# agordon/fastx_toolkit

Measured on AMD Instinct MI355X. Metric: Mreads/s (150 bp) quality-trim+filter, higher is better.
Workload: dtype u8

## Files before the change

fastx_toolkit_amd/csrc/fxg_device.h:

```cpp
#pragma once
#include <hip/hip_runtime.h>
#include <stdint.h>
#include <cstdio>
#include <cstring>

#include "../../include/fxg.h"

typedef unsigned int       u32;
typedef unsigned long long u64;
typedef unsigned int u32x4 __attribute__((ext_vector_type(4)));

#define FXG_HD __host__ __device__ __forceinline__
#define FXG_PLAN_FAIL(...) do { snprintf(err, cap, __VA_ARGS__); return FXG_E_INVALID; } while (0)
static inline int fxg_text_check_len(unsigned long long text_len, char *err, size_t cap) { if (text_len > 0xFFFFFFF0ull) FXG_PLAN_FAIL("text block too large (%llu bytes)", text_len); return FXG_OK; }
static inline bool fxg_text_lpr_ok(int lpr) { return lpr == 4 || lpr == 2; }

#if defined(FXG_ABLATION) || defined(FXG_DBG_BITS)
#define FXG_DBG(a, bit) ((a).debug & (bit))
#else
#define FXG_DBG(a, bit) 0u
#endif

#define FXG_BLOCK 256
#define FXG_WAVES (FXG_BLOCK / 64)
#ifndef FXG_TBLOCK
#define FXG_TBLOCK 256
#endif
#define FXG_TWAVES (FXG_TBLOCK / 64)
#ifndef FXG_CLIP_GATHER_K
#define FXG_CLIP_GATHER_K 4
#endif
#ifndef FXG_CLIP_DEPTH
#define FXG_CLIP_DEPTH 4u
#endif
#define FXG_CK_SLOTS 7u
#ifndef FXG_CLIP_TBLOCK
#define FXG_CLIP_TBLOCK 256
#endif
#define FXG_MAX_TILE FXG_TBLOCK
#define FXG_TICKET_GROUPS 8
#define FXG_TICKET_STRIDE 32
#define FXG_CTRL_WORDS 64

struct FxgKArgs {
    const uint8_t  *bases;
    const uint8_t  *qual;
    const uint16_t *len;
    u64  n;
// ... 37 lines not shown
    int  ft_first, ft_last;
    u32  ft_trim_end, ft_min_len;
    u32  mask_char;
    u32  nf_keep_n;
    u32  rev_dw;
    u64 *extra;
    const uint8_t  *clip_src;
    u64  clip_total;
    u32  clip_stride;
    const uint16_t *wlen;
    float *clip_ck;
    u32  clip_ck_rows;
    u32  clip_ptab_rows;
    u32  clip_ptab_stride;
    u32  clip_ptab_cols;
    u32  clip_ptab_dia1;
    char adapter[100];
    uint8_t clip_ptab_row[256];
};

__device__ __forceinline__ u32 fxg_lane() { return threadIdx.x & 63u; }

FXG_HD u32 fxg_ge_flags(u32 w, u32 K) { return (((w & 0x7f7f7f7fu) + K) | w) & 0x80808080u; }

FXG_HD u32 fxg_pack4(u32 f)
{
    u32 t = f >> 7;
    t |= t >> 7;
    t |= t >> 14;
    return t & 0xFu;
// ... 552 lines not shown
```

fastx_toolkit_amd/csrc/fxg_engine_clip.hip:

```cpp
#include "fxg_host.h"

#define FXG_CLIP_CASE_PACKED(N) case -N: return fxg_launch_tiles(c, (pl.ka.clip_global ? fxg_kernel_tiles<-N, 0, true> : fxg_kernel_tiles<-N, 0, false>), pl, ctr);
#define FXG_CLIP_CASE_GENERAL(N) case N: return fxg_launch_tiles(c, fxg_kernel_tiles<N, 0>, pl, ctr);
#define FXG_CLIP_DEFINE_UNIT(K) \
    int FXG_CLIP_UNIT_FN(K)(fxg_ctx *c, FxgPlan &pl, u64 *ctr) { switch (pl.amax) { FXG_CLIP_UNIT(K)(FXG_CLIP_CASE_PACKED, FXG_CLIP_CASE_GENERAL) default: return FXG_CLIP_NOT_MINE; } }

#ifdef FXG_CLIP_TU
FXG_CLIP_DEFINE_UNIT(FXG_CLIP_TU)
#else
FXG_CLIP_FOR_UNITS(FXG_CLIP_DEFINE_UNIT)
#endif
```

fastx_toolkit_amd/csrc/fxg_kernels.h:

```cpp
#pragma once
#include "fxg_device.h"
#include "fxg_clip_instances.h"

#define FXG_INVALID_TUPLE 0xFFFFFFFFu

#define FXG_NTALLY 16
struct FxgLds {
    u32 slot_bytes, so_ksrc, so_kidx, so_ktab;
    u32 off_scratch, off_tally, off_bm_g, off_bm_l, off_bases, off_ptab, total;
    u32 has_tab;
};
__host__ __device__ inline u32 fxg_r16(u32 x) { return (x + 15u) & ~15u; }
__host__ __device__ inline FxgLds fxg_lds_layout(u32 T, u32 stride, u32 bitmaps, u32 stage_stride, u32 nslots = 2, bool no_tab = false, u32 ptab_bytes = 0u)
{
    FxgLds l;
    l.so_ksrc = fxg_r16((T + 1) * 4);
    l.so_kidx = l.so_ksrc + fxg_r16(T * 4);
    l.so_ktab = l.so_kidx + fxg_r16(T * 2);
    l.has_tab = (stage_stride || no_tab) ? 0u : 1u;
    l.slot_bytes = l.so_ktab + (l.has_tab ? fxg_r16(((T * stride + 15) / 16 + 1) * 2) : 0u);
    u32 o = nslots * l.slot_bytes;
    l.off_scratch = o; o += fxg_r16(48 * 4);
    l.off_tally = o;   o += FXG_NTALLY * 8;
    const u32 words = (T * stride + 31) / 32 + 2;
    l.off_bm_g = o;    o += bitmaps ? fxg_r16(words * 4) * (bitmaps == 4u ? 4u : 1u) : 0;
    l.off_bm_l = bitmaps == 1u ? l.off_bm_g : o;    o += bitmaps == 2u ? fxg_r16(words * 4) : 0;
    l.off_bases = o;   o += stage_stride ? fxg_r16(T * stage_stride + 16) : 0;
    l.off_ptab = o;    o += fxg_r16(ptab_bytes);
    l.total = o;
    return l;
}

FXG_HD u32 fxg_bitmap_count(const FxgKArgs &a, bool use_q, bool clip) { return !use_q ? 0u : (clip && a.tq == a.fq) ? 1u : 2u; }

#ifdef FXG_HOST_EMULATION
FXG_HD int fxg_wave_max(int n) { return n; }
#else
__device__ __forceinline__ int fxg_wave_max(int n)
{
    int v = n;
#pragma unroll
    for (int d = 1; d < 64; d <<= 1) { const int o = __shfl_xor(v, d, 64); v = o > v ? o : v; }
// ... 111 lines not shown
#define FXG_PTAB_MAX_ROWS_K 8u

FXG_HD void fxg_ptab_row_map(const char *adapter, int alen, uint8_t (&row)[256])
{
    for (int b = 0; b < 256; ++b) row[b] = 0u;
    row[0] = 0x80u;
    u32 next = 2u;
    for (int t = 0; t < alen; ++t) {
        const u32 c = (u32)(uint8_t)adapter[t];
        if (c == (u32)'N' || row[c] != 0u) continue;
        row[c] = (uint8_t)(0x80u | next++);
    }
    row[(u32)'N'] = 0x80u | 1u;
}

FXG_HD void fxg_clip_ptab_build(const FxgKArgs &a, uint8_t *ptab, u32 tid, u32 nthreads)
{
    uint16_t *lut = reinterpret_cast<uint16_t *>(ptab);
    const int COLS = (int)a.clip_ptab_cols, A = a.alen < COLS ? a.alen : COLS;
    const u32 R = a.clip_ptab_rows, ST = a.clip_ptab_stride;
    for (u32 b = tid; b < 256u; b += nthreads) {
        const u32 e = a.clip_ptab_row[b], row = e & 0x7Fu;
        lut[b] = (uint16_t)(FXG_PTAB_LUT_BYTES + row * ST);
        if (e & 0x80u) {
            float *pv = reinterpret_cast<float *>(ptab + FXG_PTAB_LUT_BYTES + row * ST);
            u32 *sv = reinterpret_cast<u32 *>(ptab + FXG_PTAB_LUT_BYTES + (R + row) * ST);
            for (int t = 0; t < COLS; ++t) {
                const u32 tc = t < A ? (u32)(uint8_t)a.adapter[t] : 0u;
                const bool eq = tc == b, qn = b == (u32)'N', tn = tc == (u32)'N';
                pv[t] = tn ? (qn ? 0.0f : 0.1f) : (qn ? 0.1f : (eq ? 1.0f : -1.0f));
                sv[t] = (tn || qn) ? 0u : a.clip_ptab_dia1 + (eq ? 1u : 0u);
            }
        }
    }
}

#ifndef FXG_HOST_EMULATION
#define FXG_SCHED_FENCE() __builtin_amdgcn_sched_barrier(0)
// ... 119 lines not shown
#else
            const u32 w = reinterpret_cast<const u32 *>(rd)[k];
#endif
            const u32 v = w ^ 0x4E4E4E4Eu;
            const u32 z = (v - 0x01010101u) & ~v & 0x80808080u;
            const int pos = 4 * k + (int)((u32)__builtin_ctz(z | 0x80000000u) >> 3);
            first_n = (z != 0u && pos < len) ? pos : first_n;
        }
    } else {
#pragma unroll 1
        for (int k = len_u - 1; k >= 0; --k) first_n = (k < len && rd[k] == (uint8_t)'N') ? k : first_n;
    }
    return first_n;
}

template <int AMAX, bool GL = false>
FXG_HD int fxg_clip_two_pass(const FxgKArgs &a, const uint8_t *rd, int len, int rows, float &best, u32 &bw, u32 &bq, int &first_n, const bool UR = false, const uint8_t *ptab = nullptr)
{
    constexpr int C = FxgClip2<AMAX>::C;
    float S[AMAX], Sm[AMAX], P0[AMAX], P1[AMAX], P2[AMAX], CB[AMAX];
    const int A = a.alen;
#pragma unroll
    for (int t = 0; t < AMAX; ++t) { S[t] = (t <= 3) ? 0.0f : -5.0f * (float)(t - 3); Sm[t] = S[t] + -5.0f; P0[t] = P1[t] = P2[t] = CB[t] = S[t]; }
    const int early_rows = (A - 4 < rows) ? (A - 4 > 0 ? A - 4 : 0) : rows;
    const int rows_u = UR ? rows : fxg_wave_max(rows > 0 ? rows : 0);
    if (rows_u <= 0) return 0;
    float b1 = -1000000.0f;
    int q = 0, r0 = 0, bq1 = 0;
    u32 cn = 0u, gw0 = 0u, gw1 = 0u;
    int gmax = 0;
    u32 pr[16] = {}, st[16] = {}, on = 0u;
    const u32 step_off = a.clip_ptab_rows * a.clip_ptab_stride;
    const uint16_t *lut = reinterpret_cast<const uint16_t *>(ptab);
    if constexpr (GL) {
        gmax = fxg_gl_last_dword(a.clip_total, (u64)(rd - a.clip_src));
        gw0 = fxg_ld32(rd, 0, gmax); gw1 = fxg_ld32(rd, 1, gmax);
        on = lut[(gw0 >> 8) & 0xFFu];
        fxg_ptab_fetch<AMAX, false>(ptab, lut[gw0 & 0xFFu], step_off, pr, st);
    } else {
        const u32 o0 = lut[rd[0]];
        on = lut[rd[1]]; cn = rd[2];
        fxg_ptab_fetch<AMAX, false>(ptab, o0, step_off, pr, st);
    }
#define FXG_CLIP_CHUNK(EARLY, Psave, Pwin)                                                                                   \
    {                                                                                                                        \
        _Pragma("unroll") for (int t = 0; t < AMAX; ++t) Psave[t] = S[t];                                                    \
        const int q0 = q, qend = q + C < rows_u ? q + C : rows_u;                                                            \
        bool upd = false;                                                                                                    \
        _Pragma("unroll 1") for (; q < qend; ++q) {                                                                          \
            float rm;                                                                                                        \
            if constexpr (GL) {                   \
                const u32 ca = ((((q + 2) >> 2) == (q >> 2) ? gw0 : gw1) >> ((u32)((q + 2) & 3) << 3)) & 0xFFu;             \
                const u32 on2 = lut[ca];                                                                                     \
                if ((q & 3) == 3) { gw0 = gw1; gw1 = fxg_ld32(rd, (q >> 2) + 2, gmax); }                                     \
                if (!UR && q >= rows) continue;                                                                              \
                rm = fxg_clip_row_score_t<AMAX, EARLY>(A, q, S, Sm, pr, st, ptab, on, step_off);                             \
                on = on2;                                                                                                    \
            } else {                                                                                                         \
                if (!UR && q >= rows) continue;           \
                const u32 on2 = lut[cn];                                                                                     \
                cn = rd[q + 3];                                                                                              \
                rm = fxg_clip_row_score_t<AMAX, EARLY>(A, q, S, Sm, pr, st, ptab, on, step_off);                             \
                on = on2;                                                                                                    \
            }                                                                                                                \
            const bool g = rm > b1;                                                                                          \
            b1 = g ? rm : b1; bq1 = g ? q : bq1; upd = upd || g;                                                             \
        }                                                                                                                    \
        if (upd) {                                                                                                           \
            _Pragma("unroll") for (int t = 0; t < AMAX; ++t) CB[t] = Pwin[t];                                                \
            r0 = q0 - 2 * C > 0 ? q0 - 2 * C : 0;                                                                            \
        }                                                                                                                    \
    }
    static_assert(2 * C >= AMAX - 4, "early rows must end inside the first two chunks");
    FXG_CLIP_CHUNK(true, P0, P1)
    if (q < rows_u) FXG_CLIP_CHUNK(true, P1, P2)
    while (q < rows_u) {
// ... 1 lines not shown
        if (q >= rows_u) break;
        FXG_CLIP_CHUNK(false, P0, P1)
        if (q >= rows_u) break;
        FXG_CLIP_CHUNK(false, P1, P2)
    }
#undef FXG_CLIP_CHUNK
    if (rows <= 0) return 0;
    if (FXG_DBG(a, 32u)) { best = b1; bq = (u32)bq1; bw = 0u; return 0; }
    u32 W[AMAX];
#pragma unroll
    for (int t = 0; t < AMAX; ++t) { S[t] = CB[t]; Sm[t] = CB[t] + -5.0f; W[t] = ((u32)(t + 1) << 19) + FXG_PK_SZ1; }
    q = r0;
    constexpr int SPAN = FxgClip2<AMAX>::SPAN;
    const int rs = bq1 - SPAN + 1 > r0 ? bq1 - SPAN + 1 : r0;
    const int qlast = rows - 1;
#define FXG_RD_AHEAD(i) rd[GL && (i) > qlast ? qlast : (i)]
    {
        const u32 o0 = lut[rd[q]];
        on = lut[FXG_RD_AHEAD(q + 1)]; cn = FXG_RD_AHEAD(q + 2);
        fxg_ptab_fetch<AMAX, true>(ptab, o0, step_off, pr, st);
    }
    const int n0 = rs - r0, n0u = fxg_wave_max(n0);
#pragma unroll 1
    for (int i = 0; i < n0u; ++i) {
        if (i >= n0) continue;
        const u32 on2 = lut[cn];
        cn = FXG_RD_AHEAD(q + 3);
        (void)fxg_clip_row_score_t<AMAX, true, true>(A, q, S, Sm, pr, st, ptab, on, step_off);
        on = on2; ++q;
    }
    const int win = bq1 - rs, n1 = win < early_rows ? win : early_rows, n2 = win - n1;
    const int n1u = fxg_wave_max(n1), n2u = fxg_wave_max(n2);
#pragma unroll 1
    for (int i = 0; i < n1u; ++i) {
        if (i >= n1) continue;
        const u32 on2 = lut[cn];
        cn = FXG_RD_AHEAD(q + 3);
        fxg_clip_row_packed_t<AMAX, true, false>(A, q, (u32)(q - rs), S, Sm, W, best, bw, bq, pr, st, ptab, on, step_off);
        on = on2; ++q;
    }
#pragma unroll 1
    for (int i = 0; i < n2u; ++i) {
        if (i >= n2) continue;
        const u32 on2 = lut[cn];
        cn = FXG_RD_AHEAD(q + 3);
        fxg_clip_row_packed_t<AMAX, false, false>(A, q, (u32)(q - rs), S, Sm, W, best, bw, bq, pr, st, ptab, on, step_off);
        on = on2; ++q;
    }
    fxg_clip_row_packed_t<AMAX, true, true>(A, bq1, (u32)(bq1 - rs), S, Sm, W, best, bw, bq, pr, st, ptab, on, step_off);
#undef FXG_RD_AHEAD
    if (!(a.clip_flags & FXG_CLIP_KEEP_N)) first_n = fxg_clip_first_n(rd, len, UR ? len : fxg_wave_max(len), a.clip_stride, first_n);
    return rs;
}

#define FXG_K_MAT1 1u
#define FXG_K_DIA1 (1u << 7)
#define FXG_K_SZ1  (1u << 14)
#define FXG_K_START(v) ((u32)(v) << 23)
__host__ __device__ constexpr int fxg_clip_k_amin(int amax) { return amax <= 16 ? 1 : fxg_clip_bucket_below(amax) + 1; }
static_assert(fxg_clip_k_amin(16) == 1 && fxg_clip_k_amin(20) == 17 && fxg_clip_k_amin(24) == 21 && fxg_clip_k_amin(64) == 61 && fxg_clip_k_amin(72) == 65 &&
              fxg_clip_k_amin(88) == 81 && fxg_clip_k_amin(100) == 89, "a bucket's smallest adapter is the next smaller bucket + 1");
template <int AMAX> struct FxgClipK { static constexpr bool SM = AMAX <= 24; static constexpr int NSM = SM ? AMAX : 1; };

template <int AMAX, bool EARLY, bool TRACK>
FXG_HD void fxg_clip_row_kt(const FxgKArgs &a, int A, u32 c, int q, u32 vstart, float (&S)[AMAX], float (&Sm)[FxgClipK<AMAX>::NSM], u32 (&W)[AMAX],
                            float &best, u32 &bw, u32 &bq, const uint8_t *ptab)
// ... 213 lines not shown
        ++q;
    }
#pragma unroll 1
    for (int i = 0; i < n2u; ++i) {
        if (i >= n2) continue;
        fxg_clip_row_k<AMAX, false, false>(a, A, (u32)rd[q], q, (u32)(q - r0), S, Sk, W, best, bw, bq, ptab);
        ++q;
    }
    fxg_clip_row_k<AMAX, true, true>(a, A, (u32)rd[bq1], bq1, (u32)(bq1 - r0), S, Sk, W, best, bw, bq, ptab);
    if (!(a.clip_flags & FXG_CLIP_KEEP_N)) {
        first_n = fxg_clip_first_n(rd, len, UR ? len : fxg_wave_max(len), a.clip_stride, first_n);
    }
    return r0;
}

template <int AMAX, bool KFORM, bool GL = false>
FXG_HD void fxg_clip_read_packed(const FxgKArgs &a, const uint8_t *rd, int len, int rows,
                                 u32 *out_len, u32 *keep, u32 *reason, u32 *clipped, u32 *adapter_only, float *ck = nullptr, u32 cks = 0u, const bool UR = false,
                                 const uint8_t *ptab = nullptr)
{
    float best = -1000000.0f;
    u32 bw = FXG_INVALID_TUPLE, bq = 0u;
    int first_n = len, qbase = 0;
    if constexpr (!KFORM) qbase = fxg_clip_two_pass<AMAX, GL>(a, rd, len, rows, best, bw, bq, first_n, UR, ptab);
    if constexpr (KFORM) {
        int r0 = 0;
        if (ck) r0 = fxg_clip_two_pass_k<AMAX, GL>(a, rd, len, rows, ck, cks, best, bw, bq, first_n, UR, ptab);
        else fxg_clip_rows_k<AMAX>(a, rd, len, rows, best, bw, bq, first_n, UR, ptab);
        const int v = (int)(bw >> 23), matches = (int)(bw & 127u), diag = (int)((bw >> 7) & 127u);
        fxg_clip_finish(a, len, v < 256 ? r0 + v : 0, v < 256 ? 0 : v - 256, diag - matches, (int)((bw >> 14) & 511u), matches,
                        (int)bq, first_n, out_len, keep, reason, clipped, adapter_only);
        return;
    }
    const int matches = (int)(bw & 31u), diag = (int)((bw >> 14) & 31u);
    fxg_clip_finish(a, len, qbase + (int)(bw >> 24), (int)((bw >> 19) & 31u), diag - matches, (int)((bw >> 5) & 511u), matches,
                    (int)bq, first_n, out_len, keep, reason, clipped, adapter_only);
}

struct FxgCounts {
// ... 86 lines not shown
    for (u32 c = tid; c < nchunks; c += nthreads) {
        const u32 o = c << 4;
        const u64 at = tb + o;
        u32x4 v;
        if ((at & 15u) == 0u) v = fxg_window(src, (long long)at, total, 0, (int)(tbytes - o < 16u ? tbytes - o : 16u));
        else {
            u64 lo = 0, hi = 0;
            const int nb = (int)(tbytes - o < 16u ? tbytes - o : 16u);
            for (int i = 0; i < nb; ++i) { const u64 b = src[at + i]; if (i < 8) lo |= b << (8 * i); else hi |= b << (8 * (i - 8)); }
            v = (u32x4){(u32)lo, (u32)(lo >> 32), (u32)hi, (u32)(hi >> 32)};
        }
        *reinterpret_cast<u32x4 *>(sb + o) = v;
    }
}

__host__ __device__ constexpr int fxg_clip_cols(int amax) { return -amax; }
__host__ __device__ constexpr bool fxg_clip_kform(int amax) { return amax < -16; }
template <int AMAX, bool GL = false>
FXG_HD u32 fxg_decide_a(const FxgKArgs &a, const u32 *bm_g, const u32 *bm_l, const uint8_t *sb, u32 r0, u32 tid,
                        u32 *keep_out, u32 *len_out, float *ck = nullptr, u32 cks = 0u, const uint8_t *ptab = nullptr)
{
    const u32 stride = a.stride;
    const u32 rl = a.len ? (u32)a.len[r0 + tid] : a.fixed_len;
    u32 reason = FXG_R_KEPT, clipped = 0, keep = 1, curlen = rl, ao = 0;
    const int rows = a.wlen ? (int)a.wlen[r0 + tid] : (int)rl;
    if constexpr (AMAX > 0) fxg_clip_read<AMAX>(a, sb + tid * a.clip_stride, (int)rl, rows, &curlen, &keep, &reason, &clipped, &ao, !a.len && !a.wlen);
    if constexpr (AMAX < 0) {
        constexpr int COLS = fxg_clip_cols(AMAX);
        constexpr bool KF = fxg_clip_kform(AMAX);
        const uint8_t *rd = GL ? a.clip_src + (u64)(r0 + tid) * a.clip_stride : sb + tid * a.clip_stride;
        if (!a.len && !a.wlen) fxg_clip_read_packed<COLS, KF, GL>(a, rd, (int)a.fixed_len, (int)a.fixed_len, &curlen, &keep, &reason, &clipped, &ao, ck, cks, true, ptab);
        else fxg_clip_read_packed<COLS, KF, GL>(a, rd, (int)rl, rows, &curlen, &keep, &reason, &clipped, &ao, ck, cks, false, ptab);
    }
    if (keep && (a.stages & FXG_STAGE_QTRIM)) {
        const u32 k = fxg_bits_last(bm_g, tid * stride, curlen);
        curlen = k;
        if (!(k > 0 && (int)k >= a.qt_min_len)) { keep = 0; reason = FXG_R_QTRIM; }
    }
    if (keep && (a.stages & FXG_STAGE_QFILTER)) {
        const u32 low = bm_l == bm_g ? curlen - fxg_bits_count(bm_g, tid * stride, curlen) : fxg_bits_count(bm_l, tid * stride, curlen);
        int n0 = (int)curlen * a.qf_keep_pct / 100;
        if (n0 < 0) n0 = 0;
        if (a.qf_drop_all || (int)low > n0) { keep = 0; reason = FXG_R_QFILTER; }
    }
    const u32 w = (curlen & 0xFFFFu) | (keep << 16) | (reason << 17) | (clipped << 21) | (ao << FXG_RES_ADAPTER_ONLY_BIT);
    a.res[r0 + tid] = w;
    *keep_out = keep; *len_out = curlen;
// ... 150 lines not shown
#ifndef FXG_PRIO_WRITEOUT
#define FXG_PRIO_WRITEOUT 3
#endif
#ifndef FXG_PRIO_STAGING
#define FXG_PRIO_STAGING 2
#endif
#ifndef FXG_CLIP_WAVES_WIDE
#define FXG_CLIP_WAVES_WIDE 2
#endif
#ifdef FXG_CLIP_WAVES_ALL
__host__ __device__ constexpr int fxg_clip_waves(int amax) { return amax > 0 ? 1 : FXG_CLIP_WAVES_ALL; }
#else
__host__ __device__ constexpr int fxg_clip_waves(int amax) { return amax > 0 ? 1 : fxg_clip_cols(amax) <= 36 ? FXG_CLIP_WAVES : fxg_clip_cols(amax) <= 64 ? 3 : FXG_CLIP_WAVES_WIDE; }
#endif
template <int AMAX, int MODE> struct FxgTileBlock { static constexpr int threads = (MODE == 0 && AMAX < 0 && AMAX >= -16) ? FXG_CLIP_TBLOCK : FXG_TBLOCK; };
template <int AMAX, int MODE, bool GL = false>
__global__ __launch_bounds__((FxgTileBlock<AMAX, MODE>::threads), (AMAX == 0 ? FXG_MIN_WAVES : fxg_clip_waves(AMAX))) void fxg_kernel_tiles(const FxgKArgs a)
{
    extern __shared__ __attribute__((aligned(16))) unsigned char smem[];
    constexpr bool REV = (MODE == 2 || MODE == 5);
    constexpr u32 TB = (u32)FxgTileBlock<AMAX, MODE>::threads, TW = TB / 64u;
    const u32 T = a.tile_reads, stride = a.stride, tid = threadIdx.x;
    const bool use_q = (MODE == 0 && (a.stages & (FXG_STAGE_QTRIM | FXG_STAGE_QFILTER)) != 0) || MODE == 3;
    const u32 NSLOT = (MODE == 0 && AMAX != 0) ? a.depth : 2u;
    constexpr bool PTAB = MODE == 0 && fxg_clip_uses_ptab(AMAX);
    const FxgLds L = fxg_lds_layout(T, stride, MODE == 4 ? 4u : fxg_bitmap_count(a, use_q, MODE == 0 && AMAX != 0), (MODE == 0 && AMAX != 0) ? (GL ? 0u : a.clip_stride) : 0u, NSLOT, MODE == 0 && AMAX != 0, PTAB ? fxg_ptab_bytes(a.clip_ptab_rows, a.clip_ptab_stride) : 0u);
    u32 m_reads = 0, m_nt = 0, art_bad = 0;
    u32 *bm_g = reinterpret_cast<u32 *>(smem + L.off_bm_g);
    u32 *bm_l = reinterpret_cast<u32 *>(smem + L.off_bm_l);
    uint8_t *sb = smem + L.off_bases;
    u32 *scratch = reinterpret_cast<u32 *>(smem + L.off_scratch);
    u32 *s_tot = scratch + 2 * TW, *s_ticket = s_tot + 8;
    u64 *bc = reinterpret_cast<u64 *>(s_tot + 10);
    u64 *tally = reinterpret_cast<u64 *>(smem + L.off_tally);
    if (tid < FXG_NTALLY) tally[tid] = 0ull;
    if constexpr (PTAB) fxg_clip_ptab_build(a, smem + L.off_ptab, tid, TB);
#ifdef FXG_ABLATION
    u64 ph[8] = {0, 0, 0, 0, 0, 0, 0, 0}, pt = __builtin_amdgcn_s_memrealtime();
    const u64 clk_t0 = __builtin_amdgcn_s_memtime(), clk_r0 = __builtin_amdgcn_s_memrealtime();
#define FXG_TPHASE(i) do { const u64 now_ = __builtin_amdgcn_s_memrealtime(); ph[i] += now_ - pt; pt = now_; } while (0)
#else
#define FXG_TPHASE(i) do { } while (0)
#endif

    if (a.compact) {
        if (tid == 0) s_ticket[0] = atomicAdd(a.role, 1u);
        __syncthreads();
        const bool scanner = (s_ticket[0] == 0u);
        __syncthreads();
        if (scanner) { if (tid < 64) fxg_scanner(a); return; }
    }
// ... 7 lines not shown
    for (;;) {
        u64 peek = 0;
        if (tid < 64 && pend != FXG_NO_TILE && a.compact) peek = fxg_peek_prefix(a, pend);
        if (cur < a.ntiles) {
            constexpr bool TICKET_AFTER_DECISION = (MODE == 0 && AMAX != 0);
            if (!TICKET_AFTER_DECISION && tid == 0) s_ticket[tk ^ 1u] = atomicAdd(my_ticket, 1u);
            const u32 r0 = cur * T;
            const u64 left = a.n - (u64)r0;
            const u32 nreads = left < (u64)T ? (u32)left : T;
            const u64 tb = (u64)r0 * stride;
            const u32 tbytes = nreads * stride;
            unsigned char *sl = smem + slot * L.slot_bytes;
            if constexpr (MODE == 0 || MODE == 3 || MODE == 4) {
                if constexpr (MODE == 0 && AMAX != 0) __builtin_amdgcn_s_setprio(FXG_PRIO_STAGING);
                if (use_q && !FXG_DBG(a, 8u)) fxg_phase_bitmaps(a, tb, tbytes, bm_g, bm_l, tid, TB);
                if constexpr (MODE == 0 && AMAX != 0) { if (!GL && (!FXG_DBG(a, 16u) || pend == FXG_NO_TILE)) fxg_phase_stage_bases(a.clip_src, a.clip_total, (u64)r0 * a.clip_stride, nreads * a.clip_stride, sb, tid, TB); }
                if constexpr (MODE == 4) fxg_phase_census(a, tb, tbytes, fxg_census_bitmaps(bm_g, T, stride), tid, TB);
                __syncthreads();
                if constexpr (MODE == 0 && AMAX != 0) __builtin_amdgcn_s_setprio(0);
            }
            FXG_TPHASE(0);
            u32 keep = 0, olen = 0, anchor = tid * stride, word = 0;
            if (tid < nreads) {
                if constexpr (MODE == 0 && AMAX < -16) {
                    float *ck = a.clip_ck ? a.clip_ck + (size_t)blockIdx.x * ((size_t)FXG_CK_SLOTS * (u32)fxg_clip_cols(AMAX) * TB) + tid : nullptr;
                    word = fxg_decide_a<AMAX, GL>(a, bm_g, bm_l, sb, r0, tid, &keep, &olen, ck, TB, PTAB ? smem + L.off_ptab : nullptr);
                } else if constexpr (MODE == 0 && AMAX < 0) {
                    word = fxg_decide_a<AMAX, GL>(a, bm_g, bm_l, sb, r0, tid, &keep, &olen, nullptr, 0u, PTAB ? smem + L.off_ptab : nullptr);
                } else if constexpr (MODE == 0) word = fxg_decide_a<AMAX>(a, bm_g, bm_l, sb, r0, tid, &keep, &olen);
                else if constexpr (MODE == 3) { u32 nl; word = fxg_decide_mask(a, bm_l, r0, tid, &keep, &olen, &nl); m_nt += nl; m_reads += (nl != 0u); }
                else if constexpr (MODE == 4) word = fxg_decide_census(a, fxg_census_bitmaps(bm_g, T, stride), tid * stride, r0, tid, &keep, &olen, &art_bad);
                else word = fxg_decide_b<REV>(a, r0, tid, &keep, &olen, &anchor);
            }
#ifdef FXG_ABLATION
            {
                const u64 b0 = __builtin_amdgcn_s_memrealtime();
                __syncthreads();
                if ((tid & 63u) == 0u) atomicAdd(reinterpret_cast<u64 *>(a.errflag + 10) + 5, __builtin_amdgcn_s_memrealtime() - b0);
            }
#endif
            FXG_TPHASE(1);
            if (TICKET_AFTER_DECISION && tid == 0) s_ticket[tk ^ 1u] = atomicAdd(my_ticket, 1u);
            fxg_tile_tally<AMAX, MODE>(word, tid < nreads, tally);
// ... 151 lines not shown
```

fastx_toolkit_amd/csrc/fxg_plan.h:

```cpp
#pragma once
#include <cstdio>
#include <cstdlib>
#include <cstring>

#include "fxg_instances.h"
#include "fxg_knobs.h"

static_assert(fxg_clip_bucket(1) != 0 && fxg_clip_bucket(FXG_MAX_ADAPTER) != 0, "every adapter length the plan accepts needs a packed clip instance");

struct FxgPlan {
    FxgKArgs ka;
    bool group_a;
    bool clip, use_q, rev;
    bool mask, artifacts;
    int  inst;
    int  rows_nw;
    int  rows_h;
    int  amax;
    u32  lds;
    u32  block;
    u64  ck_per_wg;
};

static inline int fxg_clampi(long long v, int lo, int hi) { return v < lo ? lo : (v > hi ? hi : (int)v); }

static inline u32 fxg_pick_tile(u32 stride, bool clip, u32 block = FXG_TBLOCK, const FxgKnobs &kn = fxg_knobs_read(FXG_KNOBS_REQUEST))
{
    const u64 budget = clip ? 60ull * 1024 : 20ull * 1024;
    u32 T = block;
    if (kn.tile >= 1 && kn.tile <= (int)block && (kn.tile & (kn.tile - 1)) == 0) return (u32)kn.tile;
    while (T > 1 && (u64)T * stride > budget) T >>= 1;
    return T;
}

static inline FxgLds fxg_plan_layout(const FxgPlan *pl)
{
    const FxgKArgs &ka = pl->ka;
    return pl->group_a ? fxg_lds_layout(ka.tile_reads, ka.stride, fxg_bitmap_count(ka, pl->use_q, pl->clip), (pl->clip && !ka.clip_global) ? ka.clip_stride : 0u, pl->clip ? ka.depth : 2u, pl->clip,
                                        (pl->clip && fxg_clip_uses_ptab(pl->amax)) ? fxg_ptab_bytes(ka.clip_ptab_rows, ka.clip_ptab_stride) : 0u)
         : pl->mask ? fxg_lds_layout(ka.tile_reads, ka.stride, 2u, 0u)
         : pl->artifacts ? fxg_lds_layout(ka.tile_reads, ka.stride, 4u, 0u) : fxg_lds_layout(ka.tile_reads, ka.stride, 0u, 0u);
}
static inline u32 fxg_plan_lds(const FxgPlan *pl) { return fxg_plan_layout(pl).total; }

static inline int fxg_make_plan(const fxg_batch *in, const fxg_params *p, const fxg_out *out, FxgPlan *pl, char *err, size_t cap, u32 clip_stride = 0,
                                const FxgKnobs &kn = fxg_knobs_read(FXG_KNOBS_REQUEST))
{
    const u32 st = p->stages;
    const bool ga = (st & (FXG_STAGE_CLIP | FXG_STAGE_QTRIM | FXG_STAGE_QFILTER)) != 0;
    const bool gb = (st & (FXG_STAGE_REVCOMP | FXG_STAGE_FTRIM | FXG_STAGE_FTRIM_END)) != 0;
    const bool gm = (st & FXG_STAGE_MASK) != 0, gf = (st & (FXG_STAGE_ARTIFACTS | FXG_STAGE_NFILTER)) != 0;
    if ((int)ga + (int)gb + (int)gm + (int)gf != 1 || (st & (FXG_STAGE_ARTIFACTS | FXG_STAGE_NFILTER)) == (FXG_STAGE_ARTIFACTS | FXG_STAGE_NFILTER))
        FXG_PLAN_FAIL("unsupported stage chain 0x%x: use [CLIP][QTRIM][QFILTER], [REVCOMP][FTRIM|FTRIM_END], [MASK], [ARTIFACTS] or [NFILTER]", st);
    if (gm && !in->qual) FXG_PLAN_FAIL("fastq_masker needs qualities");
// ... 58 lines not shown
        ka.clip_ptab_dia1 = kform ? FXG_K_DIA1 : FXG_PK_DIA1;
        if (kform && ka.clip_ptab_rows > FXG_PTAB_MAX_ROWS_K) {
            pl->amax = ka.alen <= 32 ? 32 : ka.alen <= 64 ? 64 : 100;
            pl->ck_per_wg = 0;
        }
    }
    const u32 S = in->stride;
    const bool rows = ga && !pl->clip && ka.compact && kn.rows != 0 && S >= 28u && S <= (kn.rows >= 2 ? 304u : 208u);
    pl->inst = pl->clip ? FXG_INST_CLIP
             : rows ? (S <= 40u ? FXG_INST_MULTI4 : S <= 56u ? FXG_INST_MULTI3 : S < 80u ? FXG_INST_MULTI2
                       : S <= 104u ? FXG_INST_ROWS26 : S <= 152u ? FXG_INST_ROWS38 : S <= 208u ? FXG_INST_ROWS26X2 : FXG_INST_ROWS38X2)
             : ga ? FXG_INST_TILES00 : gm ? FXG_INST_TILES03 : gf ? FXG_INST_TILES04 : pl->rev ? FXG_INST_TILES02 : FXG_INST_TILES01;
    const FxgInstInfo ii = fxg_inst_info[pl->inst];
    pl->block = pl->clip ? fxg_tile_block(pl->amax, 0) : ii.block;
    pl->rows_nw = (int)ii.nw; pl->rows_h = (int)ii.h;
    ka.clip_global = 0u;
    u32 T = pl->rows_nw ? FXG_ROWS_T * ii.r / ii.h : fxg_pick_tile(pl->clip ? ka.clip_stride : in->stride, pl->clip, pl->block, kn);
    if (pl->clip && pl->amax < 0 && (pl->amax >= -16 || pl->ck_per_wg != 0) && clip_stride == 0u && (ka.clip_stride & 3u) == 0u && ((uintptr_t)ka.clip_src & 3u) == 0u) {
        ka.tile_reads = T; ka.depth = 2u;
        const bool cramped = T < pl->block || (156u * 1024u) / fxg_plan_lds(pl) < 3u;
        ka.clip_global = (kn.clip_global >= 0 ? kn.clip_global != 0 : cramped) ? 1u : 0u;
        if (ka.clip_global) T = pl->block;
    }
    const u64 ntiles = (in->n + T - 1) / T;
    if (ntiles > 0x7FFFFFFFull || in->n > 0xFFFFFFFFull) FXG_PLAN_FAIL("batch too large (%llu reads): split it", (unsigned long long)in->n);
    ka.tile_reads = T; ka.ntiles = (u32)ntiles;
    ka.rev_dw = 0u;
    if ((st & FXG_STAGE_REVCOMP) && !in->len && (T & 3u) == 0u) {
        u32 start = 0, cur = in->fixed_len;
        if (st & FXG_STAGE_FTRIM) {
            if (p->ft_last != 0 && (u32)p->ft_last < cur) cur = (u32)p->ft_last;
            if (p->ft_first != 1 && cur >= (u32)p->ft_first) { start = (u32)p->ft_first - 1u; cur -= start; }
        }
        if ((st & FXG_STAGE_FTRIM_END) && cur > p->ft_trim_end) cur -= p->ft_trim_end;
        const u32 A = (in->stride + cur) & 3u, C = (in->fixed_len - start) & 3u;
        ka.rev_dw = ((A == 0u && C != 0u) || (A == 2u && (C & 1u))) ? 1u : 0u;
    }
    if (kn.rev_dw >= 0) ka.rev_dw = (u32)kn.rev_dw;
    if (pl->inst == FXG_INST_TILES02 && ka.rev_dw) pl->inst = FXG_INST_TILES05;
    ka.depth = 2u;
    if (pl->clip && FXG_CLIP_DEPTH >= 3u) {
        const u32 cu_lds = 156u * 1024u, regs_wg = pl->block == 64u ? 16u : 4u;
        const u32 lds2 = fxg_plan_lds(pl);
        const u32 wg2 = cu_lds / lds2 < regs_wg ? cu_lds / lds2 : regs_wg;
        const u32 want = kn.clip_depth ? (u32)kn.clip_depth : FXG_CLIP_DEPTH;
        for (u32 d = want; d >= 3u; --d) {
            ka.depth = d;
            const u32 ldsd = fxg_plan_lds(pl);
            if ((cu_lds / ldsd < regs_wg ? cu_lds / ldsd : regs_wg) >= wg2) break;
            ka.depth = 2u;
        }
        if (want == 2u) ka.depth = 2u;
    }
    pl->lds = pl->rows_nw ? fxg_rows_lds(ka.stride, ii.h, ii.r) : fxg_plan_lds(pl);
    return FXG_OK;
}

static inline void fxg_plan_clip_from(FxgPlan *pl, const uint8_t *src, u32 stride, u64 total, const uint16_t *wlen)
{
    pl->ka.clip_src = src; pl->ka.clip_stride = stride; pl->ka.clip_total = total; pl->ka.wlen = wlen;
    pl->lds = fxg_plan_lds(pl);
}
static inline void fxg_plan_clip_from_batch(FxgPlan *pl, const fxg_batch *in) { fxg_plan_clip_from(pl, in->bases, in->stride, in->n * (u64)in->stride, nullptr); }

static inline int fxg_plan_request(const fxg_batch *in, const fxg_params *p, const fxg_out *out, bool hist_on, u32 hist_wcap, FxgPlan *pl, bool *hist, u32 *estride,
                                   char *err, size_t cap, const FxgKnobs &kn = fxg_knobs_read(FXG_KNOBS_REQUEST))
{
// ... 5 lines not shown
```

Before: 13200.

## Stage clip reads as 4-bit ptab codes in LDS to raise occupancy

Adds a code-tile source mode for the register two-pass adapter clip kernels (adapter width at most 16). The staging phase translates each base through the ptab row map and packs two 4-bit codes per byte in LDS. The scoring loop reads these nibbles, and the first-N scan works on the packed codes. The planner turns the mode on only when the halved base tile lets more workgroups fit per CU or avoids global fallback. The cost is extra translation work during staging, nibble extraction in the inner loop, and a more complex unaligned staging path.

```diff
diff --git a/fastx_toolkit_amd/csrc/fxg_device.h b/fastx_toolkit_amd/csrc/fxg_device.h
--- a/fastx_toolkit_amd/csrc/fxg_device.h
+++ b/fastx_toolkit_amd/csrc/fxg_device.h
@@ -32,6 +32,9 @@
 #endif
 #ifndef FXG_CLIP_DEPTH
 #define FXG_CLIP_DEPTH 4u
+#endif
+#ifndef FXG_CLIP_CODE_TILE
+#define FXG_CLIP_CODE_TILE 1
 #endif
 #define FXG_CK_SLOTS 7u
 #ifndef FXG_CLIP_TBLOCK
@@ -99,6 +102,7 @@
     u32  clip_ptab_rows;
     u32  clip_ptab_stride;
     u32  clip_ptab_cols;
+    u32  clip_codes;
     u32  clip_ptab_dia1;
     char adapter[100];
     uint8_t clip_ptab_row[256];
diff --git a/fastx_toolkit_amd/csrc/fxg_engine_clip.hip b/fastx_toolkit_amd/csrc/fxg_engine_clip.hip
--- a/fastx_toolkit_amd/csrc/fxg_engine_clip.hip
+++ b/fastx_toolkit_amd/csrc/fxg_engine_clip.hip
@@ -1,6 +1,12 @@
 #include "fxg_host.h"
 
-#define FXG_CLIP_CASE_PACKED(N) case -N: return fxg_launch_tiles(c, (pl.ka.clip_global ? fxg_kernel_tiles<-N, 0, true> : fxg_kernel_tiles<-N, 0, false>), pl, ctr);
+typedef void (*FxgTileKernel)(const FxgKArgs);
+template <int N> static FxgTileKernel fxg_clip_packed_kernel(const FxgKArgs &ka)
+{
+    if constexpr (N <= 16) { if (ka.clip_codes) return fxg_kernel_tiles<-N, 0, FXG_SRC_CODES>; }
+    return ka.clip_global ? fxg_kernel_tiles<-N, 0, FXG_SRC_GLOBAL> : fxg_kernel_tiles<-N, 0, FXG_SRC_BYTES>;
+}
+#define FXG_CLIP_CASE_PACKED(N) case -N: return fxg_launch_tiles(c, fxg_clip_packed_kernel<N>(pl.ka), pl, ctr);
 #define FXG_CLIP_CASE_GENERAL(N) case N: return fxg_launch_tiles(c, fxg_kernel_tiles<N, 0>, pl, ctr);
 #define FXG_CLIP_DEFINE_UNIT(K) \
     int FXG_CLIP_UNIT_FN(K)(fxg_ctx *c, FxgPlan &pl, u64 *ctr) { switch (pl.amax) { FXG_CLIP_UNIT(K)(FXG_CLIP_CASE_PACKED, FXG_CLIP_CASE_GENERAL) default: return FXG_CLIP_NOT_MINE; } }
diff --git a/fastx_toolkit_amd/csrc/fxg_kernels.h b/fastx_toolkit_amd/csrc/fxg_kernels.h
--- a/fastx_toolkit_amd/csrc/fxg_kernels.h
+++ b/fastx_toolkit_amd/csrc/fxg_kernels.h
@@ -11,7 +11,8 @@
     u32 has_tab;
 };
 __host__ __device__ inline u32 fxg_r16(u32 x) { return (x + 15u) & ~15u; }
-__host__ __device__ inline FxgLds fxg_lds_layout(u32 T, u32 stride, u32 bitmaps, u32 stage_stride, u32 nslots = 2, bool no_tab = false, u32 ptab_bytes = 0u)
+__host__ __device__ inline u32 fxg_code_row_bytes(u32 stride) { return (stride + 1u) / 2u; }
+__host__ __device__ inline FxgLds fxg_lds_layout(u32 T, u32 stride, u32 bitmaps, u32 stage_stride, u32 nslots = 2, bool no_tab = false, u32 ptab_bytes = 0u, bool codes = false)
 {
     FxgLds l;
     l.so_ksrc = fxg_r16((T + 1) * 4);
@@ -25,7 +26,7 @@
     const u32 words = (T * stride + 31) / 32 + 2;
     l.off_bm_g = o;    o += bitmaps ? fxg_r16(words * 4) * (bitmaps == 4u ? 4u : 1u) : 0;
     l.off_bm_l = bitmaps == 1u ? l.off_bm_g : o;    o += bitmaps == 2u ? fxg_r16(words * 4) : 0;
-    l.off_bases = o;   o += stage_stride ? fxg_r16(T * stage_stride + 16) : 0;
+    l.off_bases = o;   o += stage_stride ? fxg_r16(T * (codes ? fxg_code_row_bytes(stage_stride) : stage_stride) + 16) : 0;
     l.off_ptab = o;    o += fxg_r16(ptab_bytes);
     l.total = o;
     return l;
@@ -167,6 +168,7 @@
     row[(u32)'N'] = 0x80u | 1u;
 }
 
+template <bool CODES = false>
 FXG_HD void fxg_clip_ptab_build(const FxgKArgs &a, uint8_t *ptab, u32 tid, u32 nthreads)
 {
     uint16_t *lut = reinterpret_cast<uint16_t *>(ptab);
@@ -174,7 +176,8 @@
     const u32 R = a.clip_ptab_rows, ST = a.clip_ptab_stride;
     for (u32 b = tid; b < 256u; b += nthreads) {
         const u32 e = a.clip_ptab_row[b], row = e & 0x7Fu;
-        lut[b] = (uint16_t)(FXG_PTAB_LUT_BYTES + row * ST);
+        if constexpr (CODES) ptab[b] = (uint8_t)row;
+        else lut[b] = (uint16_t)(FXG_PTAB_LUT_BYTES + row * ST);
         if (e & 0x80u) {
             float *pv = reinterpret_cast<float *>(ptab + FXG_PTAB_LUT_BYTES + row * ST);
             u32 *sv = reinterpret_cast<u32 *>(ptab + FXG_PTAB_LUT_BYTES + (R + row) * ST);
@@ -324,10 +327,32 @@
     return first_n;
 }
 
-template <int AMAX, bool GL = false>
+#define FXG_SRC_BYTES  0
+#define FXG_SRC_GLOBAL 1
+#define FXG_SRC_CODES  2
+FXG_HD u32 fxg_code_at(const uint8_t *rd, int i) { return ((u32)rd[i >> 1] >> ((u32)(i & 1) << 2)) & 15u; }
+FXG_HD u32 fxg_code_off(u32 code) { return FXG_PTAB_LUT_BYTES + code * FXG_PTAB_ROW_BYTES; }
+
+FXG_HD int fxg_clip_first_n_codes(const uint8_t *rd, int len, int len_u, int first_n)
+{
+#pragma unroll 1
+    for (int k = (len_u + 7) / 8 - 1; k >= 0; --k) {
+        u32 w; __builtin_memcpy(&w, rd + 4 * k, 4);
+        const u32 v = w ^ 0x11111111u;
+        const u32 z = (v - 0x11111111u) & ~v & 0x88888888u;
+        const int pos = 8 * k + (int)((u32)__builtin_ctz(z | 0x80000000u) >> 2);
+        first_n = (z != 0u && pos < len) ? pos : first_n;
+    }
+    return first_n;
+}
+
+template <int AMAX, int SRC = FXG_SRC_BYTES>
 FXG_HD int fxg_clip_two_pass(const FxgKArgs &a, const uint8_t *rd, int len, int rows, float &best, u32 &bw, u32 &bq, int &first_n, const bool UR = false, const uint8_t *ptab = nullptr)
 {
     constexpr int C = FxgClip2<AMAX>::C;
+    constexpr bool GL = SRC == FXG_SRC_GLOBAL, CD = SRC == FXG_SRC_CODES;
+#define FXG_RD_BASE(i) (CD ? fxg_code_at(rd, (i)) : (u32)rd[(i)])
+#define FXG_RD_OFF(b) (CD ? fxg_code_off(b) : (u32)lut[(b)])
     float S[AMAX], Sm[AMAX], P0[AMAX], P1[AMAX], P2[AMAX], CB[AMAX];
     const int A = a.alen;
 #pragma unroll
@@ -348,8 +373,8 @@
         on = lut[(gw0 >> 8) & 0xFFu];
         fxg_ptab_fetch<AMAX, false>(ptab, lut[gw0 & 0xFFu], step_off, pr, st);
     } else {
-        const u32 o0 = lut[rd[0]];
-        on = lut[rd[1]]; cn = rd[2];
+        const u32 o0 = FXG_RD_OFF(FXG_RD_BASE(0));
+        on = FXG_RD_OFF(FXG_RD_BASE(1)); cn = FXG_RD_BASE(2);
         fxg_ptab_fetch<AMAX, false>(ptab, o0, step_off, pr, st);
     }
 #define FXG_CLIP_CHUNK(EARLY, Psave, Pwin)                                                                                   \
@@ -368,8 +393,8 @@
                 on = on2;                                                                                                    \
             } else {                                                                                                         \
                 if (!UR && q >= rows) continue;           \
-                const u32 on2 = lut[cn];                                                                                     \
-                cn = rd[q + 3];                                                                                              \
+                const u32 on2 = FXG_RD_OFF(cn);                                                                              \
+                cn = FXG_RD_BASE(q + 3);                                                                                     \
                 rm = fxg_clip_row_score_t<AMAX, EARLY>(A, q, S, Sm, pr, st, ptab, on, step_off);                             \
                 on = on2;                                                                                                    \
             }                                                                                                                \
@@ -401,17 +426,17 @@
     constexpr int SPAN = FxgClip2<AMAX>::SPAN;
     const int rs = bq1 - SPAN + 1 > r0 ? bq1 - SPAN + 1 : r0;
     const int qlast = rows - 1;
-#define FXG_RD_AHEAD(i) rd[GL && (i) > qlast ? qlast : (i)]
+#define FXG_RD_AHEAD(i) FXG_RD_BASE(GL && (i) > qlast ? qlast : (i))
     {
-        const u32 o0 = lut[rd[q]];
-        on = lut[FXG_RD_AHEAD(q + 1)]; cn = FXG_RD_AHEAD(q + 2);
+        const u32 o0 = FXG_RD_OFF(FXG_RD_BASE(q));
+        on = FXG_RD_OFF(FXG_RD_AHEAD(q + 1)); cn = FXG_RD_AHEAD(q + 2);
         fxg_ptab_fetch<AMAX, true>(ptab, o0, step_off, pr, st);
     }
     const int n0 = rs - r0, n0u = fxg_wave_max(n0);
 #pragma unroll 1
     for (int i = 0; i < n0u; ++i) {
         if (i >= n0) continue;
-        const u32 on2 = lut[cn];
+        const u32 on2 = FXG_RD_OFF(cn);
         cn = FXG_RD_AHEAD(q + 3);
         (void)fxg_clip_row_score_t<AMAX, true, true>(A, q, S, Sm, pr, st, ptab, on, step_off);
         on = on2; ++q;
@@ -421,7 +446,7 @@
 #pragma unroll 1
     for (int i = 0; i < n1u; ++i) {
         if (i >= n1) continue;
-        const u32 on2 = lut[cn];
+        const u32 on2 = FXG_RD_OFF(cn);
         cn = FXG_RD_AHEAD(q + 3);
         fxg_clip_row_packed_t<AMAX, true, false>(A, q, (u32)(q - rs), S, Sm, W, best, bw, bq, pr, st, ptab, on, step_off);
         on = on2; ++q;
@@ -429,14 +454,19 @@
 #pragma unroll 1
     for (int i = 0; i < n2u; ++i) {
         if (i >= n2) continue;
-        const u32 on2 = lut[cn];
+        const u32 on2 = FXG_RD_OFF(cn);
         cn = FXG_RD_AHEAD(q + 3);
         fxg_clip_row_packed_t<AMAX, false, false>(A, q, (u32)(q - rs), S, Sm, W, best, bw, bq, pr, st, ptab, on, step_off);
         on = on2; ++q;
     }
     fxg_clip_row_packed_t<AMAX, true, true>(A, bq1, (u32)(bq1 - rs), S, Sm, W, best, bw, bq, pr, st, ptab, on, step_off);
 #undef FXG_RD_AHEAD
-    if (!(a.clip_flags & FXG_CLIP_KEEP_N)) first_n = fxg_clip_first_n(rd, len, UR ? len : fxg_wave_max(len), a.clip_stride, first_n);
+#undef FXG_RD_BASE
+#undef FXG_RD_OFF
+    if (!(a.clip_flags & FXG_CLIP_KEEP_N)) {
+        if constexpr (CD) first_n = fxg_clip_first_n_codes(rd, len, UR ? len : fxg_wave_max(len), first_n);
+        else first_n = fxg_clip_first_n(rd, len, UR ? len : fxg_wave_max(len), a.clip_stride, first_n);
+    }
     return rs;
 }
 
@@ -680,7 +710,7 @@
     return r0;
 }
 
-template <int AMAX, bool KFORM, bool GL = false>
+template <int AMAX, bool KFORM, int SRC = FXG_SRC_BYTES>
 FXG_HD void fxg_clip_read_packed(const FxgKArgs &a, const uint8_t *rd, int len, int rows,
                                  u32 *out_len, u32 *keep, u32 *reason, u32 *clipped, u32 *adapter_only, float *ck = nullptr, u32 cks = 0u, const bool UR = false,
                                  const uint8_t *ptab = nullptr)
@@ -688,7 +718,9 @@
     float best = -1000000.0f;
     u32 bw = FXG_INVALID_TUPLE, bq = 0u;
     int first_n = len, qbase = 0;
-    if constexpr (!KFORM) qbase = fxg_clip_two_pass<AMAX, GL>(a, rd, len, rows, best, bw, bq, first_n, UR, ptab);
+    constexpr bool GL = SRC == FXG_SRC_GLOBAL;
+    static_assert(SRC != FXG_SRC_CODES || !KFORM, "the code tile serves the register two-pass instances only");
+    if constexpr (!KFORM) qbase = fxg_clip_two_pass<AMAX, SRC>(a, rd, len, rows, best, bw, bq, first_n, UR, ptab);
     if constexpr (KFORM) {
         int r0 = 0;
         if (ck) r0 = fxg_clip_two_pass_k<AMAX, GL>(a, rd, len, rows, ck, cks, best, bw, bq, first_n, UR, ptab);
@@ -805,9 +837,63 @@
     }
 }
 
+FXG_HD u32 fxg_codes8(const uint8_t *code, u32 w0, u32 w1)
+{
+    return (u32)code[w0 & 0xFFu] | ((u32)code[(w0 >> 8) & 0xFFu] << 4) | ((u32)code[(w0 >> 16) & 0xFFu] << 8) | ((u32)code[w0 >> 24] << 12) |
+           ((u32)code[w1 & 0xFFu] << 16) | ((u32)code[(w1 >> 8) & 0xFFu] << 20) | ((u32)code[(w1 >> 16) & 0xFFu] << 24) | ((u32)code[w1 >> 24] << 28);
+}
+FXG_HD u32 fxg_chunk_byte(const u32x4 &v, int i) { return (((i >> 2) == 0 ? v.x : (i >> 2) == 1 ? v.y : (i >> 2) == 2 ? v.z : v.w) >> (8 * (i & 3))) & 0xFFu; }
+
+FXG_HD void fxg_phase_stage_codes(const uint8_t *src, u64 total, u64 tb, u32 nrows, u32 stride, const uint8_t *code, uint8_t *sb, u32 tid, u32 nthreads)
+{
+    const u32 tbytes = nrows * stride, nchunks = (tbytes + 15u) >> 4, rb = fxg_code_row_bytes(stride);
+    for (u32 i = tid; i < 16u; i += nthreads) sb[nrows * rb + i] = 0u;
+    if ((stride & 1u) == 0u && (tb & 15u) == 0u && (tbytes & 15u) == 0u && tb + tbytes <= total) {
+        constexpr u32 U = 4;
+        for (u32 c0 = tid; c0 < nchunks; c0 += nthreads * U) {
+            u32x4 v[U];
+#pragma unroll
+            for (u32 u = 0; u < U; ++u) { const u32 c = c0 + u * nthreads; if (c < nchunks) v[u] = fxg_ld16(src + tb + ((u64)c << 4)); }
+#pragma unroll
+            for (u32 u = 0; u < U; ++u) {
+                const u32 c = c0 + u * nthreads;
+                if (c < nchunks) { u32 *d = reinterpret_cast<u32 *>(sb + (c << 3)); d[0] = fxg_codes8(code, v[u].x, v[u].y); d[1] = fxg_codes8(code, v[u].z, v[u].w); }
+            }
+        }
+        return;
+    }
+    for (u32 c = tid; c < nchunks; c += nthreads) {
+        const u32 o = c << 4;
+        const u64 at = tb + o;
+        const int nb = (int)(tbytes - o < 16u ? tbytes - o : 16u);
+        u32x4 v;
+        if ((at & 15u) == 0u) v = fxg_window(src, (long long)at, total, 0, nb);
+        else {
+            u64 lo = 0, hi = 0;
+            for (int i = 0; i < nb; ++i) { const u64 b = src[at + i]; if (i < 8) lo |= b << (8 * i); else hi |= b << (8 * (i - 8)); }
+            v = (u32x4){(u32)lo, (u32)(lo >> 32), (u32)hi, (u32)(hi >> 32)};
+        }
+        u32 r = o / stride, q = o - r * stride;
+#pragma unroll
+        for (int i = 0; i < 16; ++i) {
+            if (i < nb) {
+                if ((q & 1u) == 0u) {
+                    u32 h = 0u;
+                    if (q + 1u < stride) {
+                        if (i < 15) h = i + 1 < nb ? code[fxg_chunk_byte(v, i < 15 ? i + 1 : 15)] : 0u;
+                        else h = (at + 16u < total) ? code[src[at + 16u]] : 0u;
+                    }
+                    sb[r * rb + (q >> 1)] = (uint8_t)(code[fxg_chunk_byte(v, i)] | (h << 4));
+                }
+                if (++q == stride) { q = 0u; ++r; }
+            }
+        }
+    }
+}
+
 __host__ __device__ constexpr int fxg_clip_cols(int amax) { return -amax; }
 __host__ __device__ constexpr bool fxg_clip_kform(int amax) { return amax < -16; }
-template <int AMAX, bool GL = false>
+template <int AMAX, int SRC = FXG_SRC_BYTES>
 FXG_HD u32 fxg_decide_a(const FxgKArgs &a, const u32 *bm_g, const u32 *bm_l, const uint8_t *sb, u32 r0, u32 tid,
                         u32 *keep_out, u32 *len_out, float *ck = nullptr, u32 cks = 0u, const uint8_t *ptab = nullptr)
 {
@@ -819,9 +905,9 @@
     if constexpr (AMAX < 0) {
         constexpr int COLS = fxg_clip_cols(AMAX);
         constexpr bool KF = fxg_clip_kform(AMAX);
-        const uint8_t *rd = GL ? a.clip_src + (u64)(r0 + tid) * a.clip_stride : sb + tid * a.clip_stride;
-        if (!a.len && !a.wlen) fxg_clip_read_packed<COLS, KF, GL>(a, rd, (int)a.fixed_len, (int)a.fixed_len, &curlen, &keep, &reason, &clipped, &ao, ck, cks, true, ptab);
-        else fxg_clip_read_packed<COLS, KF, GL>(a, rd, (int)rl, rows, &curlen, &keep, &reason, &clipped, &ao, ck, cks, false, ptab);
+        const uint8_t *rd = SRC == FXG_SRC_GLOBAL ? a.clip_src + (u64)(r0 + tid) * a.clip_stride : sb + tid * (SRC == FXG_SRC_CODES ? fxg_code_row_bytes(a.clip_stride) : a.clip_stride);
+        if (!a.len && !a.wlen) fxg_clip_read_packed<COLS, KF, SRC>(a, rd, (int)a.fixed_len, (int)a.fixed_len, &curlen, &keep, &reason, &clipped, &ao, ck, cks, true, ptab);
+        else fxg_clip_read_packed<COLS, KF, SRC>(a, rd, (int)rl, rows, &curlen, &keep, &reason, &clipped, &ao, ck, cks, false, ptab);
     }
     if (keep && (a.stages & FXG_STAGE_QTRIM)) {
         const u32 k = fxg_bits_last(bm_g, tid * stride, curlen);
@@ -1002,17 +1088,19 @@
 __host__ __device__ constexpr int fxg_clip_waves(int amax) { return amax > 0 ? 1 : fxg_clip_cols(amax) <= 36 ? FXG_CLIP_WAVES : fxg_clip_cols(amax) <= 64 ? 3 : FXG_CLIP_WAVES_WIDE; }
 #endif
 template <int AMAX, int MODE> struct FxgTileBlock { static constexpr int threads = (MODE == 0 && AMAX < 0 && AMAX >= -16) ? FXG_CLIP_TBLOCK : FXG_TBLOCK; };
-template <int AMAX, int MODE, bool GL = false>
+template <int AMAX, int MODE, int SRC = FXG_SRC_BYTES>
 __global__ __launch_bounds__((FxgTileBlock<AMAX, MODE>::threads), (AMAX == 0 ? FXG_MIN_WAVES : fxg_clip_waves(AMAX))) void fxg_kernel_tiles(const FxgKArgs a)
 {
     extern __shared__ __attribute__((aligned(16))) unsigned char smem[];
+    constexpr bool GL = SRC == FXG_SRC_GLOBAL, CD = SRC == FXG_SRC_CODES;
+    static_assert(!CD || (MODE == 0 && AMAX < 0 && AMAX >= -16), "the code tile serves the register two-pass clip instances only");
     constexpr bool REV = (MODE == 2 || MODE == 5);
     constexpr u32 TB = (u32)FxgTileBlock<AMAX, MODE>::threads, TW = TB / 64u;
     const u32 T = a.tile_reads, stride = a.stride, tid = threadIdx.x;
     const bool use_q = (MODE == 0 && (a.stages & (FXG_STAGE_QTRIM | FXG_STAGE_QFILTER)) != 0) || MODE == 3;
     const u32 NSLOT = (MODE == 0 && AMAX != 0) ? a.depth : 2u;
     constexpr bool PTAB = MODE == 0 && fxg_clip_uses_ptab(AMAX);
-    const FxgLds L = fxg_lds_layout(T, stride, MODE == 4 ? 4u : fxg_bitmap_count(a, use_q, MODE == 0 && AMAX != 0), (MODE == 0 && AMAX != 0) ? (GL ? 0u : a.clip_stride) : 0u, NSLOT, MODE == 0 && AMAX != 0, PTAB ? fxg_ptab_bytes(a.clip_ptab_rows, a.clip_ptab_stride) : 0u);
+    const FxgLds L = fxg_lds_layout(T, stride, MODE == 4 ? 4u : fxg_bitmap_count(a, use_q, MODE == 0 && AMAX != 0), (MODE == 0 && AMAX != 0) ? (GL ? 0u : a.clip_stride) : 0u, NSLOT, MODE == 0 && AMAX != 0, PTAB ? fxg_ptab_bytes(a.clip_ptab_rows, a.clip_ptab_stride) : 0u, CD);
     u32 m_reads = 0, m_nt = 0, art_bad = 0;
     u32 *bm_g = reinterpret_cast<u32 *>(smem + L.off_bm_g);
     u32 *bm_l = reinterpret_cast<u32 *>(smem + L.off_bm_l);
@@ -1022,7 +1110,7 @@
     u64 *bc = reinterpret_cast<u64 *>(s_tot + 10);
     u64 *tally = reinterpret_cast<u64 *>(smem + L.off_tally);
     if (tid < FXG_NTALLY) tally[tid] = 0ull;
-    if constexpr (PTAB) fxg_clip_ptab_build(a, smem + L.off_ptab, tid, TB);
+    if constexpr (PTAB) fxg_clip_ptab_build<CD>(a, smem + L.off_ptab, tid, TB);
 #ifdef FXG_ABLATION
     u64 ph[8] = {0, 0, 0, 0, 0, 0, 0, 0}, pt = __builtin_amdgcn_s_memrealtime();
     const u64 clk_t0 = __builtin_amdgcn_s_memtime(), clk_r0 = __builtin_amdgcn_s_memrealtime();
@@ -1060,7 +1148,8 @@
             if constexpr (MODE == 0 || MODE == 3 || MODE == 4) {
                 if constexpr (MODE == 0 && AMAX != 0) __builtin_amdgcn_s_setprio(FXG_PRIO_STAGING);
                 if (use_q && !FXG_DBG(a, 8u)) fxg_phase_bitmaps(a, tb, tbytes, bm_g, bm_l, tid, TB);
-                if constexpr (MODE == 0 && AMAX != 0) { if (!GL && (!FXG_DBG(a, 16u) || pend == FXG_NO_TILE)) fxg_phase_stage_bases(a.clip_src, a.clip_total, (u64)r0 * a.clip_stride, nreads * a.clip_stride, sb, tid, TB); }
+                if constexpr (CD) { if (!FXG_DBG(a, 16u) || pend == FXG_NO_TILE) fxg_phase_stage_codes(a.clip_src, a.clip_total, (u64)r0 * a.clip_stride, nreads, a.clip_stride, smem + L.off_ptab, sb, tid, TB); }
+                else if constexpr (MODE == 0 && AMAX != 0) { if (!GL && (!FXG_DBG(a, 16u) || pend == FXG_NO_TILE)) fxg_phase_stage_bases(a.clip_src, a.clip_total, (u64)r0 * a.clip_stride, nreads * a.clip_stride, sb, tid, TB); }
                 if constexpr (MODE == 4) fxg_phase_census(a, tb, tbytes, fxg_census_bitmaps(bm_g, T, stride), tid, TB);
                 __syncthreads();
                 if constexpr (MODE == 0 && AMAX != 0) __builtin_amdgcn_s_setprio(0);
@@ -1070,9 +1159,9 @@
             if (tid < nreads) {
                 if constexpr (MODE == 0 && AMAX < -16) {
                     float *ck = a.clip_ck ? a.clip_ck + (size_t)blockIdx.x * ((size_t)FXG_CK_SLOTS * (u32)fxg_clip_cols(AMAX) * TB) + tid : nullptr;
-                    word = fxg_decide_a<AMAX, GL>(a, bm_g, bm_l, sb, r0, tid, &keep, &olen, ck, TB, PTAB ? smem + L.off_ptab : nullptr);
+                    word = fxg_decide_a<AMAX, SRC>(a, bm_g, bm_l, sb, r0, tid, &keep, &olen, ck, TB, PTAB ? smem + L.off_ptab : nullptr);
                 } else if constexpr (MODE == 0 && AMAX < 0) {
-                    word = fxg_decide_a<AMAX, GL>(a, bm_g, bm_l, sb, r0, tid, &keep, &olen, nullptr, 0u, PTAB ? smem + L.off_ptab : nullptr);
+                    word = fxg_decide_a<AMAX, SRC>(a, bm_g, bm_l, sb, r0, tid, &keep, &olen, nullptr, 0u, PTAB ? smem + L.off_ptab : nullptr);
                 } else if constexpr (MODE == 0) word = fxg_decide_a<AMAX>(a, bm_g, bm_l, sb, r0, tid, &keep, &olen);
                 else if constexpr (MODE == 3) { u32 nl; word = fxg_decide_mask(a, bm_l, r0, tid, &keep, &olen, &nl); m_nt += nl; m_reads += (nl != 0u); }
                 else if constexpr (MODE == 4) word = fxg_decide_census(a, fxg_census_bitmaps(bm_g, T, stride), tid * stride, r0, tid, &keep, &olen, &art_bad);
diff --git a/fastx_toolkit_amd/csrc/fxg_plan.h b/fastx_toolkit_amd/csrc/fxg_plan.h
--- a/fastx_toolkit_amd/csrc/fxg_plan.h
+++ b/fastx_toolkit_amd/csrc/fxg_plan.h
@@ -37,7 +37,7 @@
 {
     const FxgKArgs &ka = pl->ka;
     return pl->group_a ? fxg_lds_layout(ka.tile_reads, ka.stride, fxg_bitmap_count(ka, pl->use_q, pl->clip), (pl->clip && !ka.clip_global) ? ka.clip_stride : 0u, pl->clip ? ka.depth : 2u, pl->clip,
-                                        (pl->clip && fxg_clip_uses_ptab(pl->amax)) ? fxg_ptab_bytes(ka.clip_ptab_rows, ka.clip_ptab_stride) : 0u)
+                                        (pl->clip && fxg_clip_uses_ptab(pl->amax)) ? fxg_ptab_bytes(ka.clip_ptab_rows, ka.clip_ptab_stride) : 0u, pl->clip && ka.clip_codes != 0u)
          : pl->mask ? fxg_lds_layout(ka.tile_reads, ka.stride, 2u, 0u)
          : pl->artifacts ? fxg_lds_layout(ka.tile_reads, ka.stride, 4u, 0u) : fxg_lds_layout(ka.tile_reads, ka.stride, 0u, 0u);
 }
@@ -126,11 +126,19 @@
     const FxgInstInfo ii = fxg_inst_info[pl->inst];
     pl->block = pl->clip ? fxg_tile_block(pl->amax, 0) : ii.block;
     pl->rows_nw = (int)ii.nw; pl->rows_h = (int)ii.h;
+    const u32 cu_lds = 156u * 1024u, regs_wg = pl->block == 64u ? 16u : 4u;
+    const auto wg_per_cu = [&]() { const u32 l = fxg_plan_lds(pl); return cu_lds / l < regs_wg ? cu_lds / l : regs_wg; };
+#if FXG_CLIP_CODE_TILE && !defined(FXG_HOST_EMULATION)
+    const bool codes_ok = pl->clip && pl->amax < 0 && pl->amax >= -16 && clip_stride == 0u && ka.clip_ptab_rows <= 16u;
+#else
+    const bool codes_ok = false;
+#endif
     ka.clip_global = 0u;
     u32 T = pl->rows_nw ? FXG_ROWS_T * ii.r / ii.h : fxg_pick_tile(pl->clip ? ka.clip_stride : in->stride, pl->clip, pl->block, kn);
     if (pl->clip && pl->amax < 0 && (pl->amax >= -16 || pl->ck_per_wg != 0) && clip_stride == 0u && (ka.clip_stride & 3u) == 0u && ((uintptr_t)ka.clip_src & 3u) == 0u) {
         ka.tile_reads = T; ka.depth = 2u;
-        const bool cramped = T < pl->block || (156u * 1024u) / fxg_plan_lds(pl) < 3u;
+        bool cramped = T < pl->block || cu_lds / fxg_plan_lds(pl) < 3u;
+        if (cramped && codes_ok && T == pl->block) { ka.clip_codes = 1u; cramped = wg_per_cu() < regs_wg; ka.clip_codes = 0u; }
         ka.clip_global = (kn.clip_global >= 0 ? kn.clip_global != 0 : cramped) ? 1u : 0u;
         if (ka.clip_global) T = pl->block;
     }
@@ -150,19 +158,26 @@
     }
     if (kn.rev_dw >= 0) ka.rev_dw = (u32)kn.rev_dw;
     if (pl->inst == FXG_INST_TILES02 && ka.rev_dw) pl->inst = FXG_INST_TILES05;
-    ka.depth = 2u;
-    if (pl->clip && FXG_CLIP_DEPTH >= 3u) {
-        const u32 cu_lds = 156u * 1024u, regs_wg = pl->block == 64u ? 16u : 4u;
-        const u32 lds2 = fxg_plan_lds(pl);
-        const u32 wg2 = cu_lds / lds2 < regs_wg ? cu_lds / lds2 : regs_wg;
-        const u32 want = kn.clip_depth ? (u32)kn.clip_depth : FXG_CLIP_DEPTH;
-        for (u32 d = want; d >= 3u; --d) {
-            ka.depth = d;
-            const u32 ldsd = fxg_plan_lds(pl);
-            if ((cu_lds / ldsd < regs_wg ? cu_lds / ldsd : regs_wg) >= wg2) break;
-            ka.depth = 2u;
+    const auto pick_depth = [&]() {
+        ka.depth = 2u;
+        if (pl->clip && FXG_CLIP_DEPTH >= 3u) {
+            const u32 wg2 = wg_per_cu();
+            const u32 want = kn.clip_depth ? (u32)kn.clip_depth : FXG_CLIP_DEPTH;
+            for (u32 d = want; d >= 3u; --d) {
+                ka.depth = d;
+                if (wg_per_cu() >= wg2) break;
+                ka.depth = 2u;
+            }
+            if (want == 2u) ka.depth = 2u;
         }
-        if (want == 2u) ka.depth = 2u;
+        return wg_per_cu();
+    };
+    ka.clip_codes = 0u;
+    const u32 wg_bytes = pick_depth();
+    if (codes_ok && !ka.clip_global) {
+        const u32 depth_bytes = ka.depth;
+        ka.clip_codes = 1u;
+        if (pick_depth() <= wg_bytes) { ka.clip_codes = 0u; ka.depth = depth_bytes; }
     }
     pl->lds = pl->rows_nw ? fxg_rows_lds(ka.stride, ii.h, ii.r) : fxg_plan_lds(pl);
     return FXG_OK;
```

New measurement: 12940. 2.0% lower.
